# ZhekaiJin/the-Cooper-Mapper

Measured on AMD Instinct MI355X. Metric: point-residuals/s, higher is better.
Workload: dtype f32

## Files before the change

include/lslam_c.h:

```cpp
#ifndef LSLAM_C_H
#define LSLAM_C_H

#include <stddef.h>
#include <stdint.h>

#ifdef __cplusplus
extern "C" {
#endif

typedef struct lslam_ctx lslam_ctx;

typedef enum {
  LSLAM_OK = 0,
  LSLAM_TOO_FEW_REF = 1,
  LSLAM_NOT_CONVERGED = 2,
  LSLAM_LOW_SCORE = 3,
  LSLAM_LOW_PERCENT = 4,
  LSLAM_TOO_FEW_MATCHES = 5,
  LSLAM_ERR_INVALID = -1,
  LSLAM_ERR_HIP = -2,
  LSLAM_ERR_NO_MAP = -3,
  LSLAM_ERR_NO_SCAN = -4,
  LSLAM_ERR_TREE_DEPTH = -5,
  LSLAM_ERR_TREE_BUILD = -6,
// ... 474 lines not shown

enum { LSLAM_PG_PRIOR_XYZ = 0, LSLAM_PG_PRIOR_POSE = 1 };
int lslam_pg_set_priors(lslam_pg *pg, int32_t n_priors, const int32_t *vertex, const int32_t *type, const double *meas7,
                        const double *info36, const int32_t *kind, const double *delta);
int32_t lslam_pg_num_priors(const lslam_pg *pg);
int lslam_pg_prior_robust(lslam_pg *pg, const double *poses7, double *e2, double *rho, double *weight);
int lslam_g2o_read_priors(const char *path, int32_t *n_priors, int32_t *vertex, int32_t *type, double *meas7,
                          double *info36);

void *lslam_pg_stream(lslam_pg *pg);

void *lslam_stream(lslam_ctx *ctx);
void lslam_debug_sweep_launches(lslam_ctx *ctx, uint64_t counts[8]);
uint64_t lslam_debug_grid_launches(lslam_ctx *ctx);
uint64_t lslam_debug_grid_lean_launches(lslam_ctx *ctx);
uint64_t lslam_debug_grid_fine_launches(lslam_ctx *ctx);
void lslam_debug_grid_fine_info(lslam_ctx *ctx, uint64_t out[4], float *build_ms);
int lslam_debug_grid_fine_table(lslam_ctx *ctx, int which_map, int32_t rebuild, int32_t dims_out[4], float geom_out[5],
                                uint32_t *cell_start_out, size_t cap_cells, float *pts_out, size_t cap_pts);
uint64_t lslam_debug_grid_wide_launches(lslam_ctx *ctx);
void lslam_debug_grid_cells(lslam_ctx *ctx, uint64_t out[2]);
void lslam_debug_lazy_trees(lslam_ctx *ctx, uint64_t out[3]);
void lslam_debug_cert_stats(lslam_ctx *ctx, uint64_t out[3]);
void lslam_debug_grid_stats(lslam_ctx *ctx, uint64_t out[32]);
int lslam_debug_cert_state(lslam_ctx *ctx, float *q_xyz0, float *lb, size_t cap_points);

typedef struct lslam_loc lslam_loc;
enum { LSLAM_LOC_DROPPED = 1,
       LSLAM_LOC_HAS_VELOCITY = 2,
       LSLAM_LOC_POSE_RESET = 4,
// ... 201 lines not shown
```

the-cooper-mapper_amd/capi.py:

```python
import ctypes as C
import enum
import os
import subprocess

HERE = os.path.dirname(os.path.abspath(__file__))
CSRC = os.path.join(HERE, "csrc")
LIB_NAME = "liblslam_hip.so"

c_float_p = C.POINTER(C.c_float)
c_int32_p = C.POINTER(C.c_int32)
c_uint8_p = C.POINTER(C.c_uint8)


class LslamError(RuntimeError):
    def __init__(self, code, msg):
        super().__init__("lslam status %d: %s" % (code, msg))
        self.code = code


class Status(enum.IntEnum):
    OK = 0
    TOO_FEW_REF = 1
    NOT_CONVERGED = 2
    LOW_SCORE = 3
# ... 484 lines not shown
    "lslam_g2o_read_priors": (C.c_int, [C.c_char_p, c_int32_p, c_int32_p, c_int32_p, c_double_p, c_double_p]),
    "lslam_pg_stream": (C.c_void_p, [C.c_void_p]),
    "lslam_pg_kernel_from_name": (C.c_int, [C.c_char_p]),
    "lslam_icp_align": (C.c_int, [C.c_void_p, C.c_void_p, C.c_size_t, C.c_void_p, C.c_size_t, C.c_size_t, c_float_p, C.c_int32,
                                  C.c_double, C.c_double, c_double_p, c_int32_p, c_int32_p]),
    "lslam_debug_icp_step": (C.c_int, [C.c_void_p, C.c_void_p, C.c_size_t, C.c_void_p, C.c_size_t, C.c_size_t, c_float_p, C.c_double,
                                       c_int32_p, c_float_p, c_double_p, C.POINTER(LslamIcpStep)]),
    "lslam_debug_icp_fit": (C.c_int, [c_double_p, c_double_p, c_double_p, c_double_p, c_int32_p]),
    "lslam_comm_unique_id": (C.c_int, [c_uint8_p]),
    "lslam_comm_create": (C.c_int, [C.c_int, c_uint8_p, C.c_int32, C.c_int32, C.POINTER(C.c_void_p)]),
    "lslam_comm_destroy": (None, [C.c_void_p]),
    "lslam_comm_version": (C.c_int, [c_int32_p]),
    "lslam_comm_info": (C.c_int, [C.c_void_p, c_int32_p, c_int32_p]),
    "lslam_debug_grid_launches": (C.c_uint64, [C.c_void_p]),
    "lslam_debug_grid_lean_launches": (C.c_uint64, [C.c_void_p]),
    "lslam_debug_grid_fine_launches": (C.c_uint64, [C.c_void_p]),
    "lslam_debug_grid_fine_info": (None, [C.c_void_p, C.POINTER(C.c_uint64), C.POINTER(C.c_float)]),
    "lslam_debug_grid_fine_table": (C.c_int, [C.c_void_p, C.c_int, C.c_int32, c_int32_p, C.POINTER(C.c_float), C.POINTER(C.c_uint32),
                                              C.c_size_t, C.POINTER(C.c_float), C.c_size_t]),
    "lslam_debug_grid_wide_launches": (C.c_uint64, [C.c_void_p]),
    "lslam_debug_grid_cells": (None, [C.c_void_p, C.POINTER(C.c_uint64)]),
    "lslam_map_defer_trees": (C.c_int, [C.c_void_p, C.c_int32]),
    "lslam_debug_lazy_trees": (None, [C.c_void_p, C.POINTER(C.c_uint64)]),
    "lslam_comm_allreduce_f64": (C.c_int, [C.c_void_p, C.c_void_p, C.c_size_t, C.c_void_p]),
    "lslam_ctx_set_comm": (C.c_int, [C.c_void_p, C.c_void_p]),
    "lslam_pg_set_comm": (C.c_int, [C.c_void_p, C.c_void_p]),
}

COMM_ID_BYTES = 128
SC_POINT_CHUNK, SC_CAND_TILE, SC_MAX_TOP_K = 256, 64, 32
# ... 58 lines not shown
```

the-cooper-mapper_amd/csrc/lslam_api.hip:

```cpp
#include "../../include/lslam_c.h"

#include <algorithm>
#include <chrono>
#include <cmath>
#include <cstdarg>
#include <cstdio>
#include <cstdlib>
#include <cstring>
#include <condition_variable>
#include <functional>
#include <mutex>
#include <set>
#include <string>
#include <thread>

#include "lslam_internal.hpp"

using namespace lslam;

namespace {

thread_local std::string g_err;
std::mutex g_live_mu;
std::set<const lslam_ctx *> g_live;
// ... 155 lines not shown
  DevBuf<float4> od_oc, od_os, od_q, od_sel;
  DevBuf<int32_t> od_ind;
  int od_iter_hint = 6;
  DevBuf<float4> st_lm, st_obs;
  DevBuf<float> st_partials;
  DevBuf<StereoBlock> st_blocks;
  DevBuf<ProbBlocks> st_probs;
  std::vector<ProbBlocks> h_st_probs;
  DevBuf<ProbBlocks> st_noblocks;
  int32_t n_stereo = 0;
  int32_t n_st_sets = 0;
  int32_t n_st_blocks = 0;
  StereoCam st_cam{};
  uint64_t sweep_variants[SWEEP_N_VARIANTS] = {0};
  uint64_t grid_lean_launches = 0;
  GridDev kc, ks;
  uint64_t map_epoch = 0;
  uint64_t grid_epoch = ~0ull;
  float grid_cell = 0.0f;
  int grid_status = 0;
  GridDev kfc, kfs;
  uint64_t fine_epoch = ~0ull;
  float fine_cell = 0.0f;
  int fine_xsub_asked = 0;
  float fine_build_ms = 0.0f;
  uint64_t grid_fine_launches = 0;
  int env_grid_xsub = -1;
  bool defer_trees = false;
  bool trees_pending = false;
  DevBuf<uint32_t> bbox6;
// ... 227 lines not shown
    } else {
      e = launch_sweep_grid(a, jtj_mode, ctx->stream, e0, nullptr, lean);
    }
    ctx->sweep_variants[SWEEP_VARIANT_GRID]++;
    if (lean) ctx->grid_lean_launches++;
    if (e != hipSuccess) return e;
    bool planned = false;
    if (a.grid == 2) {
      e = launch_sweep_plan(a, ctx->stream, plan, true);
      if (e != hipSuccess) return e;
      planned = true;
      e = launch_sweep_wide(a, ctx->stream);
      if (e != hipSuccess) return e;
    }
    const int pass2 = a.stack_ovf ? (a.deep_tree ? SWEEP_VARIANT_DEEP_OVF : SWEEP_VARIANT_SHALLOW) : SWEEP_VARIANT_DEEP;
#ifdef LSLAM_EXP_NO_PASS2
    if (e1) return hipEventRecord(e1, ctx->stream);
    return hipSuccess;
#endif
    e = launch_sweep_queue(a, jtj_mode, ctx->stream, e1, pass2, plan, planned);
    ctx->queue_launches++;
    return e;
  }
  int v = -1;
  bool cert_launched = false;
  const bool two_pass = a.prev_q && a.need_cnt && a.bounded && a.prev_valid && !a.gc.trees && a.n_groups > 0 && a.nb_total > 0;
  hipError_t e = launch_sweep(a, jtj_mode, ctx->stream, e0, two_pass ? nullptr : e1, &v, &cert_launched);
  if (v >= 0 && v < SWEEP_N_VARIANTS) ctx->sweep_variants[v]++;
  if (e == hipSuccess && two_pass) {
    if (cert_launched) {
      e = launch_sweep_queue(a, jtj_mode, ctx->stream, e1, v, plan);
      ctx->queue_launches++;
    } else if (e1) {
      e = hipEventRecord(e1, ctx->stream);
    }
  }
// ... 121 lines not shown
  HIP_TRY(hipEventCreateWithFlags(&ctx->ev_fork, hipEventDisableTiming));
  HIP_TRY(hipEventCreateWithFlags(&ctx->ev_join, hipEventDisableTiming));
  {
    int rc = ensure_states(ctx, 1);
    if (rc) return rc;
  }
  HIP_TRY(hipEventCreate(&ctx->ev0));
  HIP_TRY(hipEventCreate(&ctx->ev1));
  (void)lslam::env_once();
  if (const char *v = std::getenv("LSLAM_KNN_CERT")) ctx->env_knn_cert = std::atoi(v);
  if (const char *v = std::getenv("LSLAM_CERT_TRY_M")) ctx->env_cert_try_m = (float)std::atof(v);
  if (const char *v = std::getenv("LSLAM_CERT_TRACK_M")) ctx->env_cert_track_m = (float)std::atof(v);
  if (const char *v = std::getenv("LSLAM_GRID_CELL")) ctx->env_grid_cell = (float)std::atof(v);
  if (const char *v = std::getenv("LSLAM_GRID_CELL_CORNER")) ctx->env_grid_cell_corner = (float)std::atof(v);
  if (const char *v = std::getenv("LSLAM_GRID_XSUB")) ctx->env_grid_xsub = std::max(1, std::min(std::atoi(v), GRID_MAX_XSUB));
  if (const char *v = std::getenv("LSLAM_DEBUG_CERT_STATS")) ctx->env_debug_cert_stats = std::atoi(v);
  if (const char *v = std::getenv("LSLAM_FORCE_STACK")) {
    if (!std::strcmp(v, "deep")) ctx->env_force_stack = SWEEP_STACK_DEEP;
    else if (!std::strcmp(v, "shallow")) ctx->env_force_stack = SWEEP_STACK_SHALLOW;
    else if (!std::strcmp(v, "auto")) ctx->env_force_stack = SWEEP_STACK_AUTO;
  }
  ctx->env_debug = lslam::env_once().debug;
  if (const char *v = std::getenv("LSLAM_SEARCH")) {
    if (!std::strcmp(v, "lane")) ctx->env_search = LSLAM_SEARCH_LANE;
    else if (!std::strcmp(v, "packet")) ctx->env_search = LSLAM_SEARCH_PACKET;
    else if (!std::strcmp(v, "grid")) ctx->env_search = LSLAM_SEARCH_GRID;
  }
  {
    std::lock_guard<std::mutex> lk(g_live_mu);
    g_live.insert(ctx);
// ... 58 lines not shown
int lslam_map_defer_trees(lslam_ctx *ctx, int32_t on) {
  int rc = check_ctx(ctx, true);
  if (rc) return rc;
  ctx->defer_trees = on != 0;
  return LSLAM_OK;
}

void lslam_debug_lazy_trees(lslam_ctx *ctx, uint64_t out[3]) {
  out[0] = ctx ? ctx->lazy_sets : 0;
  out[1] = ctx ? ctx->lazy_builds : 0;
  out[2] = ctx ? (ctx->trees_pending ? 1 : 0) : 0;
}

uint64_t lslam_debug_grid_launches(lslam_ctx *ctx) { return ctx ? ctx->sweep_variants[SWEEP_VARIANT_GRID] : 0; }
uint64_t lslam_debug_grid_lean_launches(lslam_ctx *ctx) { return ctx ? ctx->grid_lean_launches : 0; }
uint64_t lslam_debug_grid_fine_launches(lslam_ctx *ctx) { return ctx ? ctx->grid_fine_launches : 0; }
void lslam_debug_grid_fine_info(lslam_ctx *ctx, uint64_t out[4], float *build_ms) {
  const bool have = ctx && ctx->kfc.view.cell_start && ctx->kfs.view.cell_start;
  out[0] = have ? (uint64_t)ctx->kfc.view.xsub : 0;
  out[1] = have ? (uint64_t)ctx->kfs.view.xsub : 0;
  out[2] = have ? (uint64_t)ctx->kfc.n_cells : 0;
  out[3] = have ? (uint64_t)ctx->kfs.n_cells : 0;
  if (build_ms) *build_ms = have ? ctx->fine_build_ms : 0.0f;
}
uint64_t lslam_debug_grid_wide_launches(lslam_ctx *) { return 0; }
void lslam_debug_grid_cells(lslam_ctx *ctx, uint64_t out[2]) {
  out[0] = ctx && ctx->kc.view.cell_start ? (uint64_t)ctx->kc.n_cells : 0;
  out[1] = ctx && ctx->ks.view.cell_start ? (uint64_t)ctx->ks.n_cells : 0;
}

// ... 2220 lines not shown
```

the-cooper-mapper_amd/csrc/lslam_device.hpp:

```cpp
#pragma once

#include <hip/hip_runtime.h>
#include <float.h>
#include <stdint.h>

namespace lslam {

#define LSLAM_DEV __device__ __forceinline__
#ifndef LSLAM_BRANCHY_LEAF
#define LSLAM_BRANCHY_LEAF 0
#endif
#ifndef LSLAM_LEAF_COMPACT
#define LSLAM_LEAF_COMPACT 0
#endif

struct alignas(16) KdNode {
  float lo, hi;
  uint32_t c1, c2;
};

struct alignas(64) PNode {
  uint32_t c1, c2;
  float box[2][6];
  uint32_t pad[2];
// ... 6 lines not shown
struct TreeView {
  const KdNode *nodes;
  const PNode *pn;
  const float4 *pts;
  float bb_lo[3], bb_hi[3];
  int32_t n_pts, n_nodes;
  uint32_t root_ref;
};

constexpr int KD_STACK_MAX = 64;

#ifndef LSLAM_PK_DIST
#define LSLAM_PK_DIST 0
#endif
typedef float lslam_f2 __attribute__((ext_vector_type(2)));
LSLAM_DEV float dist2_xyz(float qx, float qy, float qz, const float4 &p) {
#if LSLAM_PK_DIST
  const lslam_f2 q2 = {qx, qy}, p2 = {p.x, p.y};
  const lslam_f2 d2 = q2 - p2;
  const lslam_f2 s2 = d2 * d2;
  float r = __fadd_rn(s2.x, s2.y);
  const float dz = __fsub_rn(qz, p.z);
  r = __fadd_rn(r, __fmul_rn(dz, dz));
  return r;
#else
  const float dx = __fsub_rn(qx, p.x);
  float r = __fmul_rn(dx, dx);
  const float dy = __fsub_rn(qy, p.y);
  r = __fadd_rn(r, __fmul_rn(dy, dy));
  const float dz = __fsub_rn(qz, p.z);
// ... 73 lines not shown
#else
#define TS_BEGIN
#define TS_ADD(f)
#define TS_INC(f)
#endif

#ifndef LSLAM_POPW_SHALLOW
#define LSLAM_POPW_SHALLOW 2
#endif
#ifndef LSLAM_CULL_TAKE
#define LSLAM_CULL_TAKE 0
#endif
#ifndef LSLAM_TRACK_KAPPA
#define LSLAM_TRACK_KAPPA 1.0f
#endif
template <int BLOCK, bool OVF, int LDS_DEPTH, bool TRACK = false, int POPW_SET = 0>
LSLAM_DEV void knn5_search(const TreeView &T, float qx, float qy, float qz, float (&d)[5],
                           int (&p)[5], KdStack<BLOCK, OVF, LDS_DEPTH> &stk,
#ifdef LSLAM_TRAVERSAL_STATS
                           TravStats &ts,
#endif
                           const float bound = FLT_MAX, float *lb6 = nullptr) {
  static_assert(!TRACK || (!LSLAM_LEAF_COMPACT && !LSLAM_BRANCHY_LEAF), "knn5_search<TRACK> needs the default leaf (certificates would be unsound)");
  float lb = FLT_MAX;
  constexpr int POPW = POPW_SET > 0 ? POPW_SET : ((LDS_DEPTH <= 16 && LDS_DEPTH > 0) ? LSLAM_POPW_SHALLOW : 4);
#pragma unroll
  for (int i = 0; i < 5; ++i) {
    d[i] = FLT_MAX;
    p[i] = -1;
  }
  if (T.n_pts == 0) return;
// ... 37 lines not shown
        const float e1 = v2 - nd.lo, e2 = v2 - nd.hi;
        const bool l2 = (e1 + e2) < 0.0f;
        const float c2 = l2 ? e2 * e2 : e1 * e1;
        const float n2 = (mind + c2) - (feat == 0 ? ds0 : (feat == 1 ? ds1 : ds2));
        const uint32_t r2 = l2 ? nd.c1 : nd.c2;
        if (n2 < off - 1.0f) ref = r2 ^ (node | (feat << 29));
      }
#endif
    }
    TS_ADD(t_desc)
    {
      TS_INC(n_leaf)
      const int l = (int)((ref & ~KD_LEAF) >> 4), cnt = (int)(ref & 15u);
      const float worst = fminf(d[4], bound);
      float4 pt[10];
#pragma unroll
      for (int j = 0; j < 10; ++j) pt[j] = T.pts[l + j];
#if LSLAM_LEAF_COMPACT
      {
        float dist[10];
        unsigned acc = 0;
#pragma unroll
        for (int j = 0; j < 10; ++j) {
          dist[j] = dist2_xyz(qx, qy, qz, pt[j]);
          acc |= (j < cnt && dist[j] < worst) ? (1u << j) : 0u;
        }
#ifdef LSLAM_TRAVERSAL_STATS
        ts.n_cand += __popc(acc);
        ts.n_hit += acc ? 1 : 0;
#endif
        while (__builtin_amdgcn_ballot_w64(acc != 0u) != 0ull) {
          const int j = acc ? __builtin_ctz(acc) : 0;
// ... 905 lines not shown
```

the-cooper-mapper_amd/csrc/lslam_internal.hpp:

```cpp
#pragma once

#include <hip/hip_runtime.h>
#include <stdint.h>

#include <string>
#include <vector>

#include "../../include/lslam_c.h"
#include "lslam_buf.hpp"
#include "lslam_device.hpp"
#include "lslam_grid.hpp"

#if defined(LSLAM_EXP_COUNT_NOHINT) || defined(LSLAM_EXP_LOAD2) || defined(LSLAM_EXP_LOAD_TWICE) || defined(LSLAM_EXP_NO_ACC) || \
    defined(LSLAM_EXP_NO_FIT) || defined(LSLAM_EXP_NO_PASS2) || defined(LSLAM_EXP_PROCESS_TWICE) || defined(LSLAM_EXP_SETUP_TWICE) || \
    defined(LSLAM_EXP_SECTION_CLOCK) || defined(LSLAM_EXP_SLEEP) || defined(LSLAM_EXP_PASS2_CLASS)
#define LSLAM_EXPERIMENT_BUILD 1
#else
#define LSLAM_EXPERIMENT_BUILD 0
#endif

namespace lslam {

enum : int {
  COL_ATA = 0,
// ... 191 lines not shown

enum : int { SWEEP_STACK_AUTO = 0, SWEEP_STACK_DEEP = 1, SWEEP_STACK_SHALLOW = 2 };
enum : int {
  SWEEP_VARIANT_DEEP = 0,
  SWEEP_VARIANT_DEEP_OVF = 1,
  SWEEP_VARIANT_SHALLOW = 2,
  SWEEP_VARIANT_CUBES = 3,
  SWEEP_VARIANT_CUBES_OVF = 4,
  SWEEP_VARIANT_PACKET = 5,
  SWEEP_VARIANT_GRID = 8,
  SWEEP_N_VARIANTS = 9
};
inline bool grid_sweep_lean_ok(const SweepArgs &a, int jtj_mode) {
  return jtj_mode == 1 && !a.flags_out && !a.coeff_out && !a.idx_out && a.fine_gate_c < 0.0f && a.bounded && !a.cert_stats;
}
hipError_t launch_sweep_grid(const SweepArgs &a, int jtj_mode, hipStream_t s, hipEvent_t start, hipEvent_t stop, bool lean = false, bool fine = false);
hipError_t launch_sweep_wide(const SweepArgs &a, hipStream_t s);
hipError_t launch_knn5_wide(const CellGrid &G, const float4 *q, int nq, float nf_slack, int32_t *idx, float *d2, uint8_t *undecided, hipStream_t s);
hipError_t launch_knn5_grid(const CellGrid &G, const TreeView &T, const float4 *q, int nq, int32_t *idx, float *d2,
                            uint32_t *stack_ovf, int32_t *n_unproven, hipStream_t s);

struct GridDev {
  CellGrid view{};
  size_t n_cells = 0;
  DevBuf<float4> pts, tmp_pts;
  DevBuf<uint32_t> cell_start, count, coarse;
  int32_t *err = nullptr;
  bool count_clean = false;
  hipError_t build(const TreeView &T, float cell, hipStream_t s, int *status, int xsub = 1);
  hipError_t build(const float4 *src, int n, const float lo[3], const float hi[3], float cell, hipStream_t s, int *status, bool wait = true,
                   int xsub = 1);
  void release();
};
hipError_t grid_bbox2(const float4 *const pts[2], const int n[2], uint32_t *d_box12, float lo[2][3], float hi[2][3], hipStream_t s);
hipError_t grid_unsort(const CellGrid &G, float4 *out, hipStream_t s);
hipError_t launch_compact_active(const GNState *states, const ProbBlocks *probs, int n_prob, int32_t block_base, int32_t *active_blocks,
                                 int32_t *count_out, hipStream_t s, int32_t *running_out = nullptr);
hipError_t launch_sweep_plan(const SweepArgs &a, hipStream_t s, const CertPlan &plan, bool with_prefix);
hipError_t launch_sweep_queue(const SweepArgs &a, int jtj_mode, hipStream_t s, hipEvent_t stop, int variant, const CertPlan &plan, bool planned = false);
hipError_t launch_sweep(const SweepArgs &a, int jtj_mode, hipStream_t s,
                        hipEvent_t start = nullptr, hipEvent_t stop = nullptr, int *variant = nullptr, bool *cert_launched = nullptr);
hipError_t launch_solve(const SolveArgs &a, hipStream_t s);
hipError_t launch_knn5(const TreeView &T, const float4 *q, int nq, int32_t *idx, float *d2,
                       uint32_t *stack_ovf, hipStream_t s);
hipError_t launch_knn5_packet(const TreeView &T, const float4 *q, int nq, int32_t *idx, float *d2, uint32_t *stack_ovf,
                              int32_t *n_tie, hipStream_t s);
#ifdef LSLAM_PACKET_STATS
hipError_t launch_packet_stats(const TreeView &T, const float4 *q, int nq, unsigned *out, hipStream_t s);
#endif
inline size_t stack_ovf_words(size_t n_threads, int tree_depth = KD_STACK_MAX) {
  const int levels = tree_depth + 2 < KD_STACK_MAX ? tree_depth + 2 : KD_STACK_MAX;
  return 2 * (size_t)levels * n_threads;
}
hipError_t launch_gn_step_tap(GNState *st, const float *AtA, const float *Atb, float dr, float dt,
// ... 151 lines not shown
```

the-cooper-mapper_amd/csrc/lslam_kernels.hip:

```cpp
#include <hip/hip_ext.h>

#include "lslam_internal.hpp"
#include "lslam_packet.hpp"
#include "lslam_odom_dev.hpp"
#include "lslam_solve_dev.hpp"
#include "lslam_sweep_dev.hpp"

namespace lslam {

LSLAM_DEV int xcd_remap(int b, int nb) {
  const int xcd = b & 7;
  const int q = nb >> 3, r = nb & 7;
  return (xcd < r ? xcd * (q + 1) : r * (q + 1) + (xcd - r) * q) + (b >> 3);
}

LSLAM_DEV float grid_carried_bound(const float4 &pq, const float (&sel)[3]) {
  const float ex = sel[0] - pq.x, ey = sel[1] - pq.y, ez = sel[2] - pq.z;
  const float delta = sqrtf((ex * ex + ey * ey) + ez * ez);
  const float r = (sqrtf(pq.w) + delta) * (1.0f + 1.0e-5f) + 1.0e-6f;
  const float b = r * r;
  return pq.w < 1.0e30f ? b : FLT_MAX;
}

#ifdef LSLAM_EXP_PASS2_CLASS
#ifndef LSLAM_EXP_PASS2_SPLIT
#define LSLAM_EXP_PASS2_SPLIT 1.0
#endif
__device__ unsigned long long g_pass2_hist[8];
#endif
#ifndef LSLAM_SHALLOW_OCC
#define LSLAM_SHALLOW_OCC 5
#endif
template <int BLOCK, bool OVF, bool CUBES, int LDS_DEPTH, bool PACKET, int CERT = 0, int GRIDQ = 0>
LSLAM_DEV void sweep_body(const SweepArgs &a, const int jtj_mode, const int lb, const BlockDesc &bd, const GNState *st,
                          uint32_t *stack_lds, float (*red)[NCOL], float *partial_out, const int prev_valid, const int q_item = -1) {
  constexpr int NWAVE = BLOCK / 64;
  static_assert(2 * LDS_DEPTH >= 8, "staging needs eight word rows of the stack");

  const int tid = threadIdx.x;
  const int lane = tid & 63, wave = tid >> 6;
  const uint64_t dbg_t0 = a.dbg ? __builtin_readcyclecounter() : 0;
  uint64_t dbg_t1 = 0, dbg_t2 = 0;
  const bool is_surf = bd.is_surf != 0;
  const int qi = CERT == 2 ? q_item : bd.first + tid;
  bool active = CERT == 2 ? q_item >= 0 : tid < bd.count;

  float R[9], t[3], sc[6];
  {
    static_assert(offsetof(GNState, R) == 24 && offsetof(GNState, t) == 60 && offsetof(GNState, sc) == 72, "GNState layout");
    typedef uint32_t u32x16_t __attribute__((ext_vector_type(16)));
    typedef uint32_t u32x2_t __attribute__((ext_vector_type(2)));
    u32x16_t w;
    u32x2_t w2;
    asm volatile("s_load_dwordx16 %0, %2, 0x18\n\ts_load_dwordx2 %1, %2, 0x58\n\ts_waitcnt lgkmcnt(0)"
// ... 238 lines not shown
#ifdef LSLAM_EXP_PASS2_CLASS
      if (grid) {
        if (LSLAM_EXP_PASS2_CLASS == 0) {
          const float edges[5] = {0.5f, 1.0f, 2.0f, 4.99f, 1.0e30f};
#pragma unroll
          for (int b = 0; b < 5; ++b) {
            const unsigned long long m = __ballot(active && bound < edges[b] && (b == 0 || bound >= edges[b - 1]));
            if (lane == 0 && m) atomicAdd(&g_pass2_hist[b], (unsigned long long)__popcll(m));
          }
        }
        const bool tight = bound < (float)(LSLAM_EXP_PASS2_SPLIT);
        if (LSLAM_EXP_PASS2_CLASS == 1 ? tight : (LSLAM_EXP_PASS2_CLASS == 2 ? !tight : true))
          knn5_search<BLOCK, OVF, LDS_DEPTH>(T, sel[0], sel[1], sel[2], d, p, stk, bound);
      } else
#endif
      knn5_search<BLOCK, OVF, LDS_DEPTH, false, (GRIDQ == 1 && LDS_DEPTH <= 16) ? 1 : 0>(T, sel[0], sel[1], sel[2], d, p, stk, bound);
      if ((CERT || !CUBES) && a.prev_lb) a.prev_lb[qi] = 0.0f;
    }
    if (grid) {
      if (a.bounded) a.prev_q[qi] = make_float4(sel[0], sel[1], sel[2], (p[4] >= 0 && d[4] < 5.0f) ? d[4] : FLT_MAX);
    } else if (a.bounded) {
#pragma unroll
      for (int j = 0; j < 5; ++j) a.prev_nb[(size_t)qi * 5 + j] = p[j];
    }
#endif
    }
    }
    (void)searched;
    if (a.dbg) dbg_t1 = __builtin_readcyclecounter();

    point_residual(a, bd, is_surf, (GRIDQ == 2 && a.grid == 2) ? (is_surf ? a.ks.pts : a.kc.pts) : T.pts, q, sel, d, p, sc, row, rb, kept, matched, score);
  }

  if (a.dbg) dbg_t2 = __builtin_readcyclecounter();
  block_accumulate<BLOCK, CERT == 2>(jtj_mode, is_surf, row, rb, kept, matched, score, stack_lds, red, partial_out);
  if (a.dbg && lane == 0) {
    uint64_t *o = a.dbg + ((size_t)lb * NWAVE + wave) * 4;
    o[0] = dbg_t0;
    o[1] = dbg_t1;
    o[2] = dbg_t2;
    o[3] = __builtin_readcyclecounter();
  }
}

__global__ __launch_bounds__(SOLVE_THREADS) void solve_kernel(SolveArgs a) {
  GNState *st = a.states + blockIdx.x;
  if (a.reduce_only == 2 ? !st->converged : st->done) return;
  const ProbBlocks pb = a.probs[blockIdx.x];
  const float *partials = a.partials + (size_t)pb.first_block * NCOL;
  const int nb = pb.n_blocks;
// ... 98 lines not shown
    }
    const int nch = (total + SWEEP_BLOCK - 1) / SWEEP_BLOCK;
    if (nch > 0) {
      int at = 0;
      if (lane == 0) at = atomicAdd(plan.count, nch);
      at = __shfl(at, 0, 64);
      for (int c = lane; c < nch; c += 64) plan.work[at + c] = g * CERT_GROUP + c;
    }
  }
  if (tap) {
    __syncthreads();
    if (threadIdx.x < CERT_STATS_WORDS && hist[threadIdx.x]) atomicAdd(a.cert_stats + threadIdx.x, (unsigned long long)hist[threadIdx.x]);
  }
}

template <int BLOCK, bool OVF, int LDS_DEPTH, int GRIDQ = 0>
__global__ __launch_bounds__(BLOCK) __attribute__((amdgpu_waves_per_eu(LDS_DEPTH <= 16 ? LSLAM_SHALLOW_OCC : 2))) void sweep_queue_kernel(const SweepArgs a_in, const int jtj_mode_in, const CertPlan plan) {
  __shared__ float red[BLOCK / 64][NCOL];
  __shared__ uint32_t stack_lds[2 * LDS_DEPTH * BLOCK];
  __shared__ int next_w;
  __shared__ int pre_lds[CERT_GROUP + 1];
  __shared__ int pre_wave[BLOCK / 64];
  const int n_work = *plan.count;
  for (;;) {
    if (threadIdx.x == 0) next_w = atomicAdd(plan.ticket, 1);
    __syncthreads();
    const int w = __builtin_amdgcn_readfirstlane(next_w);
    if (w >= n_work) break;
    SweepArgs a = a_in;
    int jtj_mode = jtj_mode_in;
    asm volatile("" : "+s"(a.q), "+s"(a.blocks), "+s"(a.states), "+s"(a.partials), "+s"(a.prev_nb), "+s"(a.prev_q), "+s"(a.prev_lb), "+s"(jtj_mode));
    asm volatile("" : "+s"(a.tc.nodes), "+s"(a.tc.pts), "+s"(a.ts.nodes), "+s"(a.ts.pts), "+s"(a.stack_ovf), "+s"(a.need_list), "+s"(a.need_cnt), "+s"(a.groups));
    asm volatile("" : "+s"(a.spare0), "+s"(a.spare1), "+s"(a.grid_hint));
    const int item_id = __builtin_amdgcn_readfirstlane(plan.work[w]);
    const int g = item_id / CERT_GROUP, c = item_id % CERT_GROUP;
    GroupDesc gd = a.groups[g];
    gd.first_block = __builtin_amdgcn_readfirstlane(gd.first_block);
    gd.n_blocks = __builtin_amdgcn_readfirstlane(gd.n_blocks);
    gd.prob = __builtin_amdgcn_readfirstlane(gd.prob);
    const int fb = gd.first_block - a.group_block_base;
    static_assert(CERT_GROUP <= BLOCK && (CERT_GROUP & (CERT_GROUP - 1)) == 0, "one list length per thread; the search below halves");
    {
      const int k = (int)threadIdx.x, ln = k & 63, wv = k >> 6;
      int run = k < gd.n_blocks ? (int)a.need_cnt[fb + k] : 0;
#pragma unroll
      for (int o = 1; o < 64; o <<= 1) {
        const int u = __shfl_up(run, o, 64);
        if (ln >= o) run += u;
      }
      if (CERT_GROUP > 64) {
        if (ln == 63) pre_wave[wv] = run;
        __syncthreads();
#pragma unroll
        for (int w = 0; w < BLOCK / 64; ++w) run += w < wv ? pre_wave[w] : 0;
      }
      if (k < CERT_GROUP) pre_lds[k + 1] = run;
      if (k == 0) pre_lds[0] = 0;
    }
    __syncthreads();
    const int total = pre_lds[CERT_GROUP];
    BlockDesc bd = a.blocks[fb];
    bd.prob = gd.prob;
    bd.is_surf = __builtin_amdgcn_readfirstlane(bd.is_surf);
    bd.out_base = __builtin_amdgcn_readfirstlane(bd.out_base);
    GNState *st = const_cast<GNState *>(a.states) + gd.prob;
    const int i = c * BLOCK + (int)threadIdx.x;
    int item = -1;
    if (i < total) {
      int k = 0;
#pragma unroll
      for (int step = CERT_GROUP / 2; step >= 1; step >>= 1)
        if (pre_lds[k + step] <= i) k += step;
      const int p0 = pre_lds[k];
      item = a.blocks[fb + k].first + (int)a.need_list[(size_t)(fb + k) * BLOCK + (i - p0)];
    }
    sweep_body<BLOCK, OVF, false, LDS_DEPTH, false, 2, GRIDQ>(a, jtj_mode, fb + c, bd, st, stack_lds, red, a.partials + (size_t)(fb + c) * NCOL, a.prev_valid, item);
    __syncthreads();
  }
}

hipError_t launch_sweep(const SweepArgs &a, int jtj_mode, hipStream_t s, hipEvent_t start,
                        hipEvent_t stop, int *variant, bool *cert_launched) {
  if (variant) *variant = -1;
  if (cert_launched) *cert_launched = false;
  if (a.nb_total <= 0) return hipSuccess;
  const dim3 g(a.nb_total), b(SWEEP_BLOCK);
  const bool cubes = a.gc.trees != nullptr;
#ifndef LSLAM_SHALLOW_DEPTH
#define LSLAM_SHALLOW_DEPTH 12
#endif
  constexpr int SHALLOW = LSLAM_SHALLOW_DEPTH;
// ... 29 lines not shown
    v = SWEEP_VARIANT_DEEP;
    if (cert) hipExtLaunchKernelGGL((sweep_kernel<SWEEP_BLOCK, false, false, KD_STACK_LDS, false, 1>), g, b, 0, s, start, stop, 0, a, jtj_mode);
    else hipExtLaunchKernelGGL((sweep_kernel<SWEEP_BLOCK, false, false, KD_STACK_LDS>), g, b, 0, s, start, stop, 0, a, jtj_mode);
  }
  if (variant) *variant = v;
  if (cert_launched) *cert_launched = cert && (v == SWEEP_VARIANT_SHALLOW || v == SWEEP_VARIANT_DEEP_OVF || v == SWEEP_VARIANT_DEEP);
  return hipGetLastError();
}

hipError_t launch_sweep_plan(const SweepArgs &a, hipStream_t s, const CertPlan &plan, bool with_prefix) {
  if (a.n_groups <= 0) return hipSuccess;
  hipLaunchKernelGGL(cert_plan_kernel, dim3((a.n_groups + 3) / 4 + (with_prefix ? 1 : 0)), dim3(256), 0, s, a, plan, with_prefix ? 1 : 0);
  return hipGetLastError();
}

hipError_t launch_sweep_queue(const SweepArgs &a, int jtj_mode, hipStream_t s, hipEvent_t stop, int variant, const CertPlan &plan, bool planned) {
  if (a.n_groups <= 0) return hipSuccess;
  if (!planned) hipLaunchKernelGGL(cert_plan_kernel, dim3((a.n_groups + 3) / 4), dim3(256), 0, s, a, plan, 0);
  constexpr int SHALLOW = LSLAM_SHALLOW_DEPTH;
  const long possible = a.active_blocks ? std::max<long>(a.n_active, 1) : (long)a.nb_total;
  const dim3 b(SWEEP_BLOCK);
  if (a.grid == 2) {
    const dim3 g((unsigned)std::min<long>(possible, 256 * 5));
    hipExtLaunchKernelGGL((sweep_queue_kernel<SWEEP_BLOCK, true, SHALLOW, 2>), g, b, 0, s, nullptr, stop, 0, a, jtj_mode, plan);
  } else if (variant == SWEEP_VARIANT_SHALLOW) {
    const dim3 g((unsigned)std::min<long>(possible, 256 * 5));
    if (a.grid) hipExtLaunchKernelGGL((sweep_queue_kernel<SWEEP_BLOCK, true, SHALLOW, 1>), g, b, 0, s, nullptr, stop, 0, a, jtj_mode, plan);
    else hipExtLaunchKernelGGL((sweep_queue_kernel<SWEEP_BLOCK, true, SHALLOW>), g, b, 0, s, nullptr, stop, 0, a, jtj_mode, plan);
  } else if (variant == SWEEP_VARIANT_DEEP_OVF) {
    const dim3 g((unsigned)std::min<long>(possible, 256 * 2));
    if (a.grid) hipExtLaunchKernelGGL((sweep_queue_kernel<SWEEP_BLOCK, true, KD_STACK_LDS, 1>), g, b, 0, s, nullptr, stop, 0, a, jtj_mode, plan);
    else hipExtLaunchKernelGGL((sweep_queue_kernel<SWEEP_BLOCK, true, KD_STACK_LDS>), g, b, 0, s, nullptr, stop, 0, a, jtj_mode, plan);
  } else if (variant == SWEEP_VARIANT_DEEP) {
    const dim3 g((unsigned)std::min<long>(possible, 256 * 2));
    if (a.grid) hipExtLaunchKernelGGL((sweep_queue_kernel<SWEEP_BLOCK, false, KD_STACK_LDS, 1>), g, b, 0, s, nullptr, stop, 0, a, jtj_mode, plan);
    else hipExtLaunchKernelGGL((sweep_queue_kernel<SWEEP_BLOCK, false, KD_STACK_LDS>), g, b, 0, s, nullptr, stop, 0, a, jtj_mode, plan);
  } else {
    return hipErrorInvalidValue;
  }
// ... 902 lines not shown
```

the-cooper-mapper_amd/csrc/lslam_sweep_dev.hpp:

```cpp
#pragma once

#include "lslam_internal.hpp"
#include "lslam_odom_dev.hpp"

namespace lslam {

using f32x4 = __attribute__((ext_vector_type(4))) float;

LSLAM_DEV int cube_tree_of(const CubeGridDev &g, float x, float y, float z) {
  const int gi = (int)(roundf(x / g.cube_size) + (float)g.origin[0]);
  const int gj = (int)(roundf(y / g.cube_size) + (float)g.origin[1]);
  const int gk = (int)(roundf(z / g.cube_size) + (float)g.origin[2]);
  if (0 <= gi && gi < g.dims[0] && 0 <= gj && gj < g.dims[1] && 0 <= gk && gk < g.dims[2])
    return g.cell_tree[gi + gj * g.dims[0] + gk * g.dims[0] * g.dims[1]];
  return -1;
}

template <bool GIVEN = false>
LSLAM_DEV void point_residual(const SweepArgs &a, const BlockDesc &bd, const bool is_surf, const float4 *P, const float4 &q,
                              const float (&sel)[3], const float (&d)[5], const int (&p)[5], const float (&sc)[6],
                              float (&row)[6], float &rb, float &kept, float &matched, float &score,
                              const float (*given)[15] = nullptr, const bool use_given = false) {
  float coeff[4] = {0, 0, 0, 0};
  unsigned flag = 0;
// ... 63 lines not shown
  }
  if (a.flags_out) {
    const int gi = bd.out_base + __float_as_int(q.w);
    a.flags_out[gi] = (uint8_t)flag;
    if (a.coeff_out) a.coeff_out[gi] = make_float4(coeff[0], coeff[1], coeff[2], coeff[3]);
    if (a.idx_out) {
#pragma unroll
      for (int j = 0; j < 5; ++j) {
        a.idx_out[gi * 5 + j] = p[j] >= 0 ? __float_as_int(P[p[j]].w) : -1;
        a.d2_out[gi * 5 + j] = d[j];
      }
    }
  }
}

template <int BLOCK, bool ADD, int PAD = 0>
LSLAM_DEV void block_accumulate(const int jtj_mode, const bool is_surf, const float (&row)[6], const float rb, const float kept,
                                const float matched, const float score, uint32_t *stage, float (*red)[NCOL], float *partial_out) {
  constexpr int NWAVE = BLOCK / 64;
  const int tid = threadIdx.x;
  const int lane = tid & 63, wave = tid >> 6;
  float v[NCOL];
#pragma unroll
  for (int i = 0; i < NCOL; ++i) v[i] = 0.0f;

#ifdef LSLAM_EXP_NO_ACC
  if (false) {
#else
  if (jtj_mode == 1) {
#endif
    constexpr int ST = BLOCK + PAD;
    float *jr = reinterpret_cast<float *>(stage) + wave * 64;
#pragma unroll
    for (int c = 0; c < 6; ++c) jr[c * ST + lane] = row[c];
    jr[6 * ST + lane] = rb;
// ... 60 lines not shown
```

the-cooper-mapper_amd/scan_match.py:

```python
import ctypes as C

import numpy as np

from .capi import (LslamError, LslamMapInfo, LslamOpts, LslamStats, Status, c_float_p, c_int32_p,
                   c_uint8_p, load_library)


def _cloud(a):
    a = np.ascontiguousarray(a, dtype=np.float32)
    if a.ndim != 2 or a.shape[1] < 3:
        raise ValueError("cloud must be (n, >=3) float32, got %r" % (a.shape,))
    return a, a.shape[1] * 4


def _vp(a):
    return a.ctypes.data_as(C.c_void_p)


def _fp(a):
    return a.ctypes.data_as(c_float_p)


class Comm:

# ... 88 lines not shown
        return dict(zip(SWEEP_VARIANTS, (int(v) for v in out)))

    def defer_trees(self, on=True):
        self._check(self.lib.lslam_map_defer_trees(self.h, int(bool(on))))

    def lazy_trees(self):
        out = (C.c_uint64 * 3)()
        self.lib.lslam_debug_lazy_trees(self.h, out)
        return int(out[0]), int(out[1]), bool(out[2])

    def grid_launches(self):
        return int(self.lib.lslam_debug_grid_launches(self.h))

    def grid_lean_launches(self):
        return int(self.lib.lslam_debug_grid_lean_launches(self.h))

    def grid_fine_launches(self):
        return int(self.lib.lslam_debug_grid_fine_launches(self.h))

    def grid_fine_info(self):
        out = (C.c_uint64 * 4)()
        ms = C.c_float(0.0)
        self.lib.lslam_debug_grid_fine_info(self.h, out, C.byref(ms))
        return dict(xsub=(int(out[0]), int(out[1])), cells=(int(out[2]), int(out[3])), build_ms=float(ms.value))

    def grid_fine_table(self, which_map, rebuild=False):
        dims = (C.c_int32 * 4)()
        geom = (C.c_float * 5)()
        n = self.lib.lslam_debug_grid_fine_table(self.h, which_map, 1 if rebuild else 0, dims, geom, None, 0, None, 0)
        if n < 0:
# ... 448 lines not shown
```

Baseline: 14.93 billion.

## Add lean specialization of grid sweep's second-pass queue kernel

Adds a LEAN template instantiation of the queue sweep kernel for the grid path's shallow-overflow second pass. It constant-folds the debug, flags, coefficient and cert-stats options, loads leaf points as 12-byte xyz, and uses a higher waves-per-EU target so register pressure drops and occupancy rises. The path is on by default when its preconditions hold, and LSLAM_QUEUE_LEAN turns it off. The risks are register spills at the higher occupancy target and a slightly different launch grid size.

```diff
diff --git a/include/lslam_c.h b/include/lslam_c.h
--- a/include/lslam_c.h
+++ b/include/lslam_c.h
@@ -512,6 +512,7 @@
 void lslam_debug_sweep_launches(lslam_ctx *ctx, uint64_t counts[8]);
 uint64_t lslam_debug_grid_launches(lslam_ctx *ctx);
 uint64_t lslam_debug_grid_lean_launches(lslam_ctx *ctx);
+uint64_t lslam_debug_queue_lean_launches(lslam_ctx *ctx);
 uint64_t lslam_debug_grid_fine_launches(lslam_ctx *ctx);
 void lslam_debug_grid_fine_info(lslam_ctx *ctx, uint64_t out[4], float *build_ms);
 int lslam_debug_grid_fine_table(lslam_ctx *ctx, int which_map, int32_t rebuild, int32_t dims_out[4], float geom_out[5],
diff --git a/the-cooper-mapper_amd/capi.py b/the-cooper-mapper_amd/capi.py
--- a/the-cooper-mapper_amd/capi.py
+++ b/the-cooper-mapper_amd/capi.py
@@ -522,6 +522,7 @@
     "lslam_comm_info": (C.c_int, [C.c_void_p, c_int32_p, c_int32_p]),
     "lslam_debug_grid_launches": (C.c_uint64, [C.c_void_p]),
     "lslam_debug_grid_lean_launches": (C.c_uint64, [C.c_void_p]),
+    "lslam_debug_queue_lean_launches": (C.c_uint64, [C.c_void_p]),
     "lslam_debug_grid_fine_launches": (C.c_uint64, [C.c_void_p]),
     "lslam_debug_grid_fine_info": (None, [C.c_void_p, C.POINTER(C.c_uint64), C.POINTER(C.c_float)]),
     "lslam_debug_grid_fine_table": (C.c_int, [C.c_void_p, C.c_int, C.c_int32, c_int32_p, C.POINTER(C.c_float), C.POINTER(C.c_uint32),
diff --git a/the-cooper-mapper_amd/csrc/lslam_api.hip b/the-cooper-mapper_amd/csrc/lslam_api.hip
--- a/the-cooper-mapper_amd/csrc/lslam_api.hip
+++ b/the-cooper-mapper_amd/csrc/lslam_api.hip
@@ -193,6 +193,8 @@
   StereoCam st_cam{};
   uint64_t sweep_variants[SWEEP_N_VARIANTS] = {0};
   uint64_t grid_lean_launches = 0;
+  uint64_t queue_lean_launches = 0;
+  bool env_queue_lean = true;
   GridDev kc, ks;
   uint64_t map_epoch = 0;
   uint64_t grid_epoch = ~0ull;
@@ -450,12 +452,14 @@
       if (e != hipSuccess) return e;
     }
     const int pass2 = a.stack_ovf ? (a.deep_tree ? SWEEP_VARIANT_DEEP_OVF : SWEEP_VARIANT_SHALLOW) : SWEEP_VARIANT_DEEP;
+    const bool lean2 = lean && ctx->env_queue_lean && pass2 == SWEEP_VARIANT_SHALLOW && grid_queue_lean_ok(a, jtj_mode);
 #ifdef LSLAM_EXP_NO_PASS2
     if (e1) return hipEventRecord(e1, ctx->stream);
     return hipSuccess;
 #endif
-    e = launch_sweep_queue(a, jtj_mode, ctx->stream, e1, pass2, plan, planned);
+    e = launch_sweep_queue(a, jtj_mode, ctx->stream, e1, pass2, plan, planned, lean2);
     ctx->queue_launches++;
+    if (lean2) ctx->queue_lean_launches++;
     return e;
   }
   int v = -1;
@@ -607,6 +611,7 @@
   if (const char *v = std::getenv("LSLAM_GRID_CELL")) ctx->env_grid_cell = (float)std::atof(v);
   if (const char *v = std::getenv("LSLAM_GRID_CELL_CORNER")) ctx->env_grid_cell_corner = (float)std::atof(v);
   if (const char *v = std::getenv("LSLAM_GRID_XSUB")) ctx->env_grid_xsub = std::max(1, std::min(std::atoi(v), GRID_MAX_XSUB));
+  if (const char *v = std::getenv("LSLAM_QUEUE_LEAN")) ctx->env_queue_lean = std::atoi(v) != 0;
   if (const char *v = std::getenv("LSLAM_DEBUG_CERT_STATS")) ctx->env_debug_cert_stats = std::atoi(v);
   if (const char *v = std::getenv("LSLAM_FORCE_STACK")) {
     if (!std::strcmp(v, "deep")) ctx->env_force_stack = SWEEP_STACK_DEEP;
@@ -695,6 +700,7 @@
 
 uint64_t lslam_debug_grid_launches(lslam_ctx *ctx) { return ctx ? ctx->sweep_variants[SWEEP_VARIANT_GRID] : 0; }
 uint64_t lslam_debug_grid_lean_launches(lslam_ctx *ctx) { return ctx ? ctx->grid_lean_launches : 0; }
+uint64_t lslam_debug_queue_lean_launches(lslam_ctx *ctx) { return ctx ? ctx->queue_lean_launches : 0; }
 uint64_t lslam_debug_grid_fine_launches(lslam_ctx *ctx) { return ctx ? ctx->grid_fine_launches : 0; }
 void lslam_debug_grid_fine_info(lslam_ctx *ctx, uint64_t out[4], float *build_ms) {
   const bool have = ctx && ctx->kfc.view.cell_start && ctx->kfs.view.cell_start;
diff --git a/the-cooper-mapper_amd/csrc/lslam_device.hpp b/the-cooper-mapper_amd/csrc/lslam_device.hpp
--- a/the-cooper-mapper_amd/csrc/lslam_device.hpp
+++ b/the-cooper-mapper_amd/csrc/lslam_device.hpp
@@ -44,6 +44,7 @@
 #define LSLAM_PK_DIST 0
 #endif
 typedef float lslam_f2 __attribute__((ext_vector_type(2)));
+struct alignas(16) f32x3_ld { float x, y, z; };
 LSLAM_DEV float dist2_xyz(float qx, float qy, float qz, const float4 &p) {
 #if LSLAM_PK_DIST
   const lslam_f2 q2 = {qx, qy}, p2 = {p.x, p.y};
@@ -147,7 +148,7 @@
 #ifndef LSLAM_TRACK_KAPPA
 #define LSLAM_TRACK_KAPPA 1.0f
 #endif
-template <int BLOCK, bool OVF, int LDS_DEPTH, bool TRACK = false, int POPW_SET = 0>
+template <int BLOCK, bool OVF, int LDS_DEPTH, bool TRACK = false, int POPW_SET = 0, bool XYZ = false>
 LSLAM_DEV void knn5_search(const TreeView &T, float qx, float qy, float qz, float (&d)[5],
                            int (&p)[5], KdStack<BLOCK, OVF, LDS_DEPTH> &stk,
 #ifdef LSLAM_TRAVERSAL_STATS
@@ -215,8 +216,16 @@
       const int l = (int)((ref & ~KD_LEAF) >> 4), cnt = (int)(ref & 15u);
       const float worst = fminf(d[4], bound);
       float4 pt[10];
+      if constexpr (XYZ) {
+#pragma unroll
+        for (int j = 0; j < 10; ++j) {
+          const f32x3_ld v = *reinterpret_cast<const f32x3_ld *>(T.pts + l + j);
+          pt[j] = make_float4(v.x, v.y, v.z, 0.0f);
+        }
+      } else {
 #pragma unroll
       for (int j = 0; j < 10; ++j) pt[j] = T.pts[l + j];
+      }
 #if LSLAM_LEAF_COMPACT
       {
         float dist[10];
diff --git a/the-cooper-mapper_amd/csrc/lslam_internal.hpp b/the-cooper-mapper_amd/csrc/lslam_internal.hpp
--- a/the-cooper-mapper_amd/csrc/lslam_internal.hpp
+++ b/the-cooper-mapper_amd/csrc/lslam_internal.hpp
@@ -229,6 +229,13 @@
 inline bool grid_sweep_lean_ok(const SweepArgs &a, int jtj_mode) {
   return jtj_mode == 1 && !a.flags_out && !a.coeff_out && !a.idx_out && a.fine_gate_c < 0.0f && a.bounded && !a.cert_stats;
 }
+inline bool grid_queue_lean_ok(const SweepArgs &a, int jtj_mode) {
+#ifdef LSLAM_TRAVERSAL_STATS
+  return false;
+#else
+  return grid_sweep_lean_ok(a, jtj_mode) && a.grid == 1 && !a.dbg && !a.prev_lb && a.stack_ovf && !a.deep_tree;
+#endif
+}
 hipError_t launch_sweep_grid(const SweepArgs &a, int jtj_mode, hipStream_t s, hipEvent_t start, hipEvent_t stop, bool lean = false, bool fine = false);
 hipError_t launch_sweep_wide(const SweepArgs &a, hipStream_t s);
 hipError_t launch_knn5_wide(const CellGrid &G, const float4 *q, int nq, float nf_slack, int32_t *idx, float *d2, uint8_t *undecided, hipStream_t s);
@@ -252,7 +259,8 @@
 hipError_t launch_compact_active(const GNState *states, const ProbBlocks *probs, int n_prob, int32_t block_base, int32_t *active_blocks,
                                  int32_t *count_out, hipStream_t s, int32_t *running_out = nullptr);
 hipError_t launch_sweep_plan(const SweepArgs &a, hipStream_t s, const CertPlan &plan, bool with_prefix);
-hipError_t launch_sweep_queue(const SweepArgs &a, int jtj_mode, hipStream_t s, hipEvent_t stop, int variant, const CertPlan &plan, bool planned = false);
+hipError_t launch_sweep_queue(const SweepArgs &a, int jtj_mode, hipStream_t s, hipEvent_t stop, int variant, const CertPlan &plan, bool planned = false,
+                              bool lean = false);
 hipError_t launch_sweep(const SweepArgs &a, int jtj_mode, hipStream_t s,
                         hipEvent_t start = nullptr, hipEvent_t stop = nullptr, int *variant = nullptr, bool *cert_launched = nullptr);
 hipError_t launch_solve(const SolveArgs &a, hipStream_t s);
diff --git a/the-cooper-mapper_amd/csrc/lslam_kernels.hip b/the-cooper-mapper_amd/csrc/lslam_kernels.hip
--- a/the-cooper-mapper_amd/csrc/lslam_kernels.hip
+++ b/the-cooper-mapper_amd/csrc/lslam_kernels.hip
@@ -31,13 +31,16 @@
 #ifndef LSLAM_SHALLOW_OCC
 #define LSLAM_SHALLOW_OCC 5
 #endif
-template <int BLOCK, bool OVF, bool CUBES, int LDS_DEPTH, bool PACKET, int CERT = 0, int GRIDQ = 0>
+template <int BLOCK, bool OVF, bool CUBES, int LDS_DEPTH, bool PACKET, int CERT = 0, int GRIDQ = 0, bool LEAN = false>
 LSLAM_DEV void sweep_body(const SweepArgs &a, const int jtj_mode, const int lb, const BlockDesc &bd, const GNState *st,
                           uint32_t *stack_lds, float (*red)[NCOL], float *partial_out, const int prev_valid, const int q_item = -1) {
   constexpr int NWAVE = BLOCK / 64;
   static_assert(2 * LDS_DEPTH >= 8, "staging needs eight word rows of the stack");
-
-  const int tid = threadIdx.x;
+  static_assert(!LEAN || (CERT == 2 && GRIDQ == 1 && !PACKET && !CUBES), "LEAN is the grid sweep's second pass over whole-map trees");
+
+  int tid_v = threadIdx.x;
+  if constexpr (LEAN) asm volatile("" : "+v"(tid_v));
+  const int tid = tid_v;
   const int lane = tid & 63, wave = tid >> 6;
   const uint64_t dbg_t0 = a.dbg ? __builtin_readcyclecounter() : 0;
   uint64_t dbg_t1 = 0, dbg_t2 = 0;
@@ -306,8 +309,8 @@
           knn5_search<BLOCK, OVF, LDS_DEPTH>(T, sel[0], sel[1], sel[2], d, p, stk, bound);
       } else
 #endif
-      knn5_search<BLOCK, OVF, LDS_DEPTH, false, (GRIDQ == 1 && LDS_DEPTH <= 16) ? 1 : 0>(T, sel[0], sel[1], sel[2], d, p, stk, bound);
-      if ((CERT || !CUBES) && a.prev_lb) a.prev_lb[qi] = 0.0f;
+      knn5_search<BLOCK, OVF, LDS_DEPTH, false, (GRIDQ == 1 && LDS_DEPTH <= 16) ? 1 : 0, LEAN>(T, sel[0], sel[1], sel[2], d, p, stk, bound);
+      if (!LEAN && (CERT || !CUBES) && a.prev_lb) a.prev_lb[qi] = 0.0f;
     }
     if (grid) {
       if (a.bounded) a.prev_q[qi] = make_float4(sel[0], sel[1], sel[2], (p[4] >= 0 && d[4] < 5.0f) ? d[4] : FLT_MAX);
@@ -325,7 +328,7 @@
   }
 
   if (a.dbg) dbg_t2 = __builtin_readcyclecounter();
-  block_accumulate<BLOCK, CERT == 2>(jtj_mode, is_surf, row, rb, kept, matched, score, stack_lds, red, partial_out);
+  block_accumulate<BLOCK, CERT == 2, 0, LEAN>(jtj_mode, is_surf, row, rb, kept, matched, score, stack_lds, red, partial_out);
   if (a.dbg && lane == 0) {
     uint64_t *o = a.dbg + ((size_t)lb * NWAVE + wave) * 4;
     o[0] = dbg_t0;
@@ -454,8 +457,12 @@
   }
 }
 
-template <int BLOCK, bool OVF, int LDS_DEPTH, int GRIDQ = 0>
-__global__ __launch_bounds__(BLOCK) __attribute__((amdgpu_waves_per_eu(LDS_DEPTH <= 16 ? LSLAM_SHALLOW_OCC : 2))) void sweep_queue_kernel(const SweepArgs a_in, const int jtj_mode_in, const CertPlan plan) {
+#ifndef LSLAM_QUEUE_LEAN_OCC
+#define LSLAM_QUEUE_LEAN_OCC 6
+#endif
+template <int BLOCK, bool OVF, int LDS_DEPTH, int GRIDQ = 0, bool LEAN = false>
+__global__ __launch_bounds__(BLOCK) __attribute__((amdgpu_waves_per_eu(LEAN ? LSLAM_QUEUE_LEAN_OCC : (LDS_DEPTH <= 16 ? LSLAM_SHALLOW_OCC : 2)))) void sweep_queue_kernel(const SweepArgs a_in, const int jtj_mode_in, const CertPlan plan) {
+  static_assert(!LEAN || GRIDQ == 1, "LEAN is an instantiation of the grid sweep's second pass over trees");
   __shared__ float red[BLOCK / 64][NCOL];
   __shared__ uint32_t stack_lds[2 * LDS_DEPTH * BLOCK];
   __shared__ int next_w;
@@ -467,11 +474,28 @@
     __syncthreads();
     const int w = __builtin_amdgcn_readfirstlane(next_w);
     if (w >= n_work) break;
+    int tid_k = (int)threadIdx.x;
+    if constexpr (LEAN) asm volatile("" : "+v"(tid_k));
     SweepArgs a = a_in;
     int jtj_mode = jtj_mode_in;
+    if constexpr (LEAN) {
+      jtj_mode = 1;
+      a.flags_out = nullptr;
+      a.coeff_out = nullptr;
+      a.idx_out = nullptr;
+      a.fine_gate_c = -1.0f;
+      a.bounded = 1;
+      a.cert_stats = nullptr;
+      a.dbg = nullptr;
+      a.prev_lb = nullptr;
+      asm volatile("" : "+s"(a.q), "+s"(a.blocks), "+s"(a.states), "+s"(a.partials), "+s"(a.prev_q));
+      asm volatile("" : "+s"(a.tc.nodes), "+s"(a.tc.pts), "+s"(a.ts.nodes), "+s"(a.ts.pts), "+s"(a.stack_ovf), "+s"(a.need_list), "+s"(a.need_cnt), "+s"(a.groups));
+      asm volatile("" : "+s"(a.grid_hint));
+    } else {
     asm volatile("" : "+s"(a.q), "+s"(a.blocks), "+s"(a.states), "+s"(a.partials), "+s"(a.prev_nb), "+s"(a.prev_q), "+s"(a.prev_lb), "+s"(jtj_mode));
     asm volatile("" : "+s"(a.tc.nodes), "+s"(a.tc.pts), "+s"(a.ts.nodes), "+s"(a.ts.pts), "+s"(a.stack_ovf), "+s"(a.need_list), "+s"(a.need_cnt), "+s"(a.groups));
     asm volatile("" : "+s"(a.spare0), "+s"(a.spare1), "+s"(a.grid_hint));
+    }
     const int item_id = __builtin_amdgcn_readfirstlane(plan.work[w]);
     const int g = item_id / CERT_GROUP, c = item_id % CERT_GROUP;
     GroupDesc gd = a.groups[g];
@@ -481,7 +505,7 @@
     const int fb = gd.first_block - a.group_block_base;
     static_assert(CERT_GROUP <= BLOCK && (CERT_GROUP & (CERT_GROUP - 1)) == 0, "one list length per thread; the search below halves");
     {
-      const int k = (int)threadIdx.x, ln = k & 63, wv = k >> 6;
+      const int k = tid_k, ln = k & 63, wv = k >> 6;
       int run = k < gd.n_blocks ? (int)a.need_cnt[fb + k] : 0;
 #pragma unroll
       for (int o = 1; o < 64; o <<= 1) {
@@ -504,7 +528,7 @@
     bd.is_surf = __builtin_amdgcn_readfirstlane(bd.is_surf);
     bd.out_base = __builtin_amdgcn_readfirstlane(bd.out_base);
     GNState *st = const_cast<GNState *>(a.states) + gd.prob;
-    const int i = c * BLOCK + (int)threadIdx.x;
+    const int i = c * BLOCK + tid_k;
     int item = -1;
     if (i < total) {
       int k = 0;
@@ -514,7 +538,7 @@
       const int p0 = pre_lds[k];
       item = a.blocks[fb + k].first + (int)a.need_list[(size_t)(fb + k) * BLOCK + (i - p0)];
     }
-    sweep_body<BLOCK, OVF, false, LDS_DEPTH, false, 2, GRIDQ>(a, jtj_mode, fb + c, bd, st, stack_lds, red, a.partials + (size_t)(fb + c) * NCOL, a.prev_valid, item);
+    sweep_body<BLOCK, OVF, false, LDS_DEPTH, false, 2, GRIDQ, LEAN>(a, jtj_mode, fb + c, bd, st, stack_lds, red, a.partials + (size_t)(fb + c) * NCOL, a.prev_valid, item);
     __syncthreads();
   }
 }
@@ -574,8 +598,9 @@
   return hipGetLastError();
 }
 
-hipError_t launch_sweep_queue(const SweepArgs &a, int jtj_mode, hipStream_t s, hipEvent_t stop, int variant, const CertPlan &plan, bool planned) {
+hipError_t launch_sweep_queue(const SweepArgs &a, int jtj_mode, hipStream_t s, hipEvent_t stop, int variant, const CertPlan &plan, bool planned, bool lean) {
   if (a.n_groups <= 0) return hipSuccess;
+  if (lean && !(grid_queue_lean_ok(a, jtj_mode) && variant == SWEEP_VARIANT_SHALLOW)) return hipErrorInvalidValue;
   if (!planned) hipLaunchKernelGGL(cert_plan_kernel, dim3((a.n_groups + 3) / 4), dim3(256), 0, s, a, plan, 0);
   constexpr int SHALLOW = LSLAM_SHALLOW_DEPTH;
   const long possible = a.active_blocks ? std::max<long>(a.n_active, 1) : (long)a.nb_total;
@@ -583,6 +608,9 @@
   if (a.grid == 2) {
     const dim3 g((unsigned)std::min<long>(possible, 256 * 5));
     hipExtLaunchKernelGGL((sweep_queue_kernel<SWEEP_BLOCK, true, SHALLOW, 2>), g, b, 0, s, nullptr, stop, 0, a, jtj_mode, plan);
+  } else if (lean) {
+    const dim3 g((unsigned)std::min<long>(possible, 256 * LSLAM_QUEUE_LEAN_OCC));
+    hipExtLaunchKernelGGL((sweep_queue_kernel<SWEEP_BLOCK, true, SHALLOW, 1, true>), g, b, 0, s, nullptr, stop, 0, a, jtj_mode, plan);
   } else if (variant == SWEEP_VARIANT_SHALLOW) {
     const dim3 g((unsigned)std::min<long>(possible, 256 * 5));
     if (a.grid) hipExtLaunchKernelGGL((sweep_queue_kernel<SWEEP_BLOCK, true, SHALLOW, 1>), g, b, 0, s, nullptr, stop, 0, a, jtj_mode, plan);
diff --git a/the-cooper-mapper_amd/csrc/lslam_sweep_dev.hpp b/the-cooper-mapper_amd/csrc/lslam_sweep_dev.hpp
--- a/the-cooper-mapper_amd/csrc/lslam_sweep_dev.hpp
+++ b/the-cooper-mapper_amd/csrc/lslam_sweep_dev.hpp
@@ -101,11 +101,13 @@
   }
 }
 
-template <int BLOCK, bool ADD, int PAD = 0>
+template <int BLOCK, bool ADD, int PAD = 0, bool FRESH_TID = false>
 LSLAM_DEV void block_accumulate(const int jtj_mode, const bool is_surf, const float (&row)[6], const float rb, const float kept,
                                 const float matched, const float score, uint32_t *stage, float (*red)[NCOL], float *partial_out) {
   constexpr int NWAVE = BLOCK / 64;
-  const int tid = threadIdx.x;
+  int tid_v = threadIdx.x;
+  if constexpr (FRESH_TID) asm volatile("" : "+v"(tid_v));
+  const int tid = tid_v;
   const int lane = tid & 63, wave = tid >> 6;
   float v[NCOL];
 #pragma unroll
diff --git a/the-cooper-mapper_amd/scan_match.py b/the-cooper-mapper_amd/scan_match.py
--- a/the-cooper-mapper_amd/scan_match.py
+++ b/the-cooper-mapper_amd/scan_match.py
@@ -126,6 +126,9 @@
 
     def grid_lean_launches(self):
         return int(self.lib.lslam_debug_grid_lean_launches(self.h))
+
+    def queue_lean_launches(self):
+        return int(self.lib.lslam_debug_queue_lean_launches(self.h))
 
     def grid_fine_launches(self):
         return int(self.lib.lslam_debug_grid_fine_launches(self.h))
```

Measured after the change: 15.29 billion, median of 6. 1.02x the previous value.
